# EricSteinberger/PokerRL

Measured on AMD Instinct MI355X. Metric: CFR+ node-updates/sec on FHP public tree, higher is better.
Workload: dtype f32

## Files before the change

include/pokerrl_hip.h:

```cpp
#ifndef POKERRL_HIP_H
#define POKERRL_HIP_H

#include <stdint.h>

#ifdef __cplusplus
extern "C" {
#endif

#define PRL_MAX_BET_SIZES 96

#define PRL_OK 0
#define PRL_ERR_ARG (-1)
#define PRL_ERR_NO_DEVICE (-2)
#define PRL_ERR_HIP (-3)
#define PRL_ERR_UNSUPPORTED (-4)
#define PRL_ERR_OOM (-5)
#define PRL_ERR_STATE (-6)

typedef struct PrlRules {
    int32_t n_hole_cards;
    int32_t n_ranks;
    int32_t n_suits;
    int32_t n_cards;
    int32_t range_size;
// ... 214 lines not shown
int32_t prl_solver_time_iterations_ex(prl_solver_t* solver, int32_t n, float* out_ms, float* out_pass_ms, int32_t* out_n_pass);

int32_t prl_solver_time_evaluations(prl_solver_t* solver, int32_t n, float* out_ms, float* out_pass_ms, int32_t* out_n_pass);

enum {
    PRL_SF_REACH = 0,
    PRL_SF_EV = 1,
    PRL_SF_EV_BR = 2,
    PRL_SF_STRATEGY = 3,
    PRL_SF_STRAT_F64 = 4,
    PRL_SF_REGRET = 5,
    PRL_SF_AVG = 6,
    PRL_SF_AVG_F64 = 7,
    PRL_SF_AVG_SUM = 8,
    PRL_SF_BR_IDX = 9,
    PRL_SF_EXPL_HISTORY = 10,
    PRL_SF_ITER = 11,
    PRL_SF_CONSTANTS = 12,
    PRL_SF_BYTES_ALLOCATED = 13,
    PRL_SF_ENGINE = 14,
    PRL_SF_GRAPH_REPLAY = 15,
    PRL_SF_EXCHANGES = 17,
    PRL_SF_VMM_RANGES = 18,
    PRL_SF_EXPLICIT_STRATEGY = 16
};
int32_t prl_solver_get(prl_solver_t* solver, int32_t field, void* out);
int32_t prl_solver_set_strategy_device(prl_solver_t* solver, const prl_tree_t* tree, const float* d_probs, int32_t n_actions);
int32_t prl_solver_get_cols(prl_solver_t* solver, int32_t field, int64_t col_begin, int64_t n_cols, void* out);

int32_t prl_lbr_checkdown_equity(const PrlRules* rules, const int8_t* board_dealt, int32_t n_dealt, const int8_t* lbr_hand,
                                 const float* ranges, int32_t n_q, float* out_wp);

int32_t prl_lbr_batch_run(const PrlGame* lbr_game, const PrlGame* agent_game, const PrlRules* rules, int32_t n_envs, int32_t agent_seat,
                          int32_t check_to_round, int32_t agent_kind, uint32_t agent_seed, uint32_t episode_base, double reward_scalar,
                          double ev_normalizer, const int8_t* cards, float* out_winnings, uint64_t* out_stats4, float* out_device_ms);

int32_t prl_h2h_batch_run(const PrlGame* game, const PrlRules* rules, int32_t n_envs, int32_t ref_seat, int32_t ref_kind, uint32_t ref_seed,
                          int32_t opp_kind, uint32_t opp_seed, uint32_t episode_base, double reward_scalar, double ev_normalizer,
                          const int8_t* cards, float* out_winnings, uint64_t* out_stats2, float* out_device_ms);

typedef struct PrlPolicyTable prl_policy_table_t;
prl_policy_table_t* prl_policy_table_create(const uint64_t* keys, const int32_t* rows, uint32_t capacity, const float* probs, int32_t n_rows,
                                            int32_t n_actions, int32_t range_size, uint32_t key_seed);
void prl_policy_table_destroy(prl_policy_table_t* table);
int32_t prl_policy_table_probe(const prl_policy_table_t* table, int32_t n, const uint32_t* key_lo, const uint32_t* key_hi, const int32_t* action,
                               const int32_t* hand, int32_t* out_row, float* out_prob);
// ... 23 lines not shown
```

pokerrl_amd/_native.py:

```python
import ctypes
import os

import numpy as np

_HERE = os.path.dirname(os.path.abspath(__file__))
EXCHANGE_FN = ctypes.CFUNCTYPE(ctypes.c_int32, ctypes.c_void_p, ctypes.c_void_p, ctypes.c_void_p, ctypes.c_uint64)
LIB_PATH = os.environ.get("POKERRL_AMD_LIB", os.path.join(_HERE, "lib", "libpokerrl_hip.so"))

PRL_MAX_BET_SIZES = 96


class NativeError(RuntimeError):
    status = None


ERR_ARG, ERR_NO_DEVICE, ERR_HIP, ERR_UNSUPPORTED, ERR_OOM, ERR_STATE = -1, -2, -3, -4, -5, -6


class PrlRules(ctypes.Structure):
    _fields_ = [
        ("n_hole_cards", ctypes.c_int32), ("n_ranks", ctypes.c_int32), ("n_suits", ctypes.c_int32),
        ("n_cards", ctypes.c_int32), ("range_size", ctypes.c_int32), ("n_rounds", ctypes.c_int32),
        ("board_cards_in_round", ctypes.c_int32 * 4), ("n_board_cards", ctypes.c_int32),
        ("btn_first_postflop", ctypes.c_int32), ("rank_rule", ctypes.c_int32),
# ... 499 lines not shown
        L.prl_tree_observations_device.restype = ctypes.c_int32
        check(L.prl_tree_observations_device(self._h, int(kind), 1 if invert else 0, _ptr(idx), _ptr(off), len(idx), None if fo is None else _ptr(fo),
                                              int(row_dim), int(n_rows), ctypes.c_void_p(int(d_out)), ctypes.c_void_p(int(d_legal or 0)), int(n_actions)), L)

    def obs_stats(self):
        out = np.zeros(4, np.float64)
        self._L.prl_tree_obs_stats.argtypes = [ctypes.c_void_p, ctypes.c_void_p]
        self._L.prl_tree_obs_stats.restype = ctypes.c_int32
        check(self._L.prl_tree_obs_stats(self._h, _ptr(out)), self._L)
        return dict(state_bytes=int(out[0]), states_ms=float(out[1]), obs_ms=float(out[2]), obs_bytes=int(out[3]))

    def __del__(self):
        try:
            if self._h:
                self._L.prl_tree_destroy(self._h)
                self._h = None
        except Exception:
            pass


OBS_VANILLA, OBS_HISTORY, OBS_FLAT_HU_LIMIT = 0, 1, 2

SF = dict(reach=0, ev=1, ev_br=2, strategy=3, strat_f64=4, regret=5, avg=6, avg_f64=7, avg_sum=8, br_idx=9,
          expl_history=10, iter=11, constants=12, bytes_allocated=13, engine=14, graph_replay=15, explicit_strategy=16, exchanges=17, vmm_ranges=18)
VARIANTS = {"vanilla": 0, "plus": 1, "linear": 2}
ENGINES = {"auto": 0, "levels": 1, "fused": 2}


class NativeSolver:

    def __init__(self, tree, variant, delay=0, engine="auto", _lib=None, shard=None, avg_dtype="f64", place=None, probe_iters=4, board_mult=None,
                 symmetrize=False):
        self._L = _lib or tree._L
        self.placement_ms, self.placement_chosen = None, None
        if _lib is None and self._L is lib():
            require_device()
        self.tree = tree
        self._h = ctypes.c_void_p()
        v = VARIANTS[variant] if isinstance(variant, str) else int(variant)
        e = ENGINES[engine] if isinstance(engine, str) else int(engine)
        self._exchange_cb = None
        if board_mult is not None and shard is not None:
            raise ValueError("weighted boards (board_mult=): one GPU -- not with shard=")
        if symmetrize and board_mult is None:
            raise ValueError("symmetrize= goes with board_mult= (suit-class representatives and their orbit sizes)")
        if shard is not None and isinstance(shard[0], str):
            assert shard[0] == "rccl"
# ... 210 lines not shown

        th = [threading.Thread(target=work, args=(n,), daemon=True) for n in names]
        for t in th:
            t.start()
        try:
            for c0 in range(0, self.n_cols, cols_per_piece):
                for n in names:
                    qs[n].put(self.get_cols(n, c0, min(cols_per_piece, self.n_cols - c0)))
        finally:
            for n in names:
                qs[n].put(None)
            for t in th:
                t.join()
        return {n: h.hexdigest() for n, h in hs.items()}

    def get(self, name):
        n, c, R = self.n_nodes, self.n_cols, self.R
        shape, dtype = {
            "reach": ((n, 2, R), np.float32), "ev": ((n, 2, R), np.float32), "ev_br": ((n, 2, R), np.float32),
            "strategy": ((c, R), np.float64), "strat_f64": ((n,), np.uint8), "regret": ((c, R), np.float32),
            "avg": ((c, R), np.float64), "avg_f64": ((n,), np.uint8), "avg_sum": ((c, R), np.float32),
            "br_idx": ((n, R), np.int32), "constants": ((2,), np.float32), "bytes_allocated": ((1,), np.int64),
            "explicit_strategy": ((1,), np.int32), "exchanges": ((1,), np.int64), "vmm_ranges": ((2,), np.int64),
        }.get(name, (None, None))
        if name == "expl_history":
            shape, dtype = (self.iter + 1, 2), np.float32
        out = np.zeros(shape, dtype)
        self._call("prl_solver_get", SF[name], _ptr(out))
        return out
```

pokerrl_amd/csrc/prl_fhp.h:

```cpp
#pragma once
#include "prl_defs.h"
#include "prl_solver_types.h"
#include "prl_tree.h"

enum { PRL_SRC_REGRET = 0, PRL_SRC_UNIFORM64 = 1, PRL_SRC_ARR64 = 2, PRL_SRC_ARR32 = 3,
       PRL_SRC_STRAT32 = 4 ,
       PRL_SRC_AVGF32 = 5  };
enum { PRL_FHP_UPDATE0 = 0, PRL_FHP_UPDATE1 = 1, PRL_FHP_EVAL = 2, PRL_FHP_UPDATE0_EVAL = 3, PRL_FHP_UPDATE0_BR = 4, PRL_FHP_UPDATE1_EVAL1 = 5,
       PRL_FHP_EVAL0 = 6 };
constexpr bool prl_fhp_runs_seat(int mode, int p) {
    return mode == PRL_FHP_EVAL || mode == PRL_FHP_UPDATE0_EVAL ? true
         : (mode == PRL_FHP_UPDATE1 || mode == PRL_FHP_UPDATE1_EVAL1) ? p == 1 : p == 0;
}
constexpr bool prl_fhp_updates(int mode, int p) {
    return p == 0 ? (mode == PRL_FHP_UPDATE0 || mode == PRL_FHP_UPDATE0_EVAL || mode == PRL_FHP_UPDATE0_BR)
                  : (mode == PRL_FHP_UPDATE1 || mode == PRL_FHP_UPDATE1_EVAL1);
}
constexpr bool prl_fhp_with_br(int mode) { return mode >= PRL_FHP_EVAL; }
constexpr int prl_fhp_out_width(int mode) {
    return mode == PRL_FHP_UPDATE1_EVAL1 ? 3
         : (prl_fhp_runs_seat(mode, 0) && prl_fhp_runs_seat(mode, 1) ? 2 : 1) * (prl_fhp_with_br(mode) ? 2 : 1);
}

#define PRL_FHP_MAX_NODES 40
// ... 85 lines not shown

struct PrlFhpShapeDesc {
    int32_t n_nodes, n_cols, n_dec;
    int32_t kind[PRL_FHP_MAX_NODES], actor[PRL_FHP_MAX_NODES], nch[PRL_FHP_MAX_NODES], parent[PRL_FHP_MAX_NODES], col0[PRL_FHP_MAX_NODES],
        folder[PRL_FHP_MAX_NODES];
    int32_t dec_nch[PRL_FHP_MAX_DEC], dec_col0[PRL_FHP_MAX_DEC];
};
template <class D>
inline PrlFhpShapeDesc prl_fhp_describe() {
    PrlFhpShapeDesc d = {};
    d.n_nodes = D::N_NODES; d.n_cols = D::N_COLS; d.n_dec = D::N_DEC;
    static_assert(D::N_NODES <= PRL_FHP_MAX_NODES && D::N_DEC <= PRL_FHP_MAX_DEC, "enlarge PRL_FHP_MAX_*");
    for (int n = 0; n < D::N_NODES; ++n) {
        d.kind[n] = D::kind(n); d.actor[n] = D::actor(n); d.nch[n] = D::nch(n); d.parent[n] = D::parent(n); d.col0[n] = D::col0(n);
        d.folder[n] = D::folder(n);
    }
    for (int j = 0; j < D::N_DEC; ++j) { d.dec_nch[j] = D::nch(D::dec_node(j)); d.dec_col0[j] = D::col0(D::dec_node(j)); }
    return d;
}
enum { PRL_FHP_SHAPE_15 = 0, PRL_FHP_SHAPE_9 = 1, PRL_FHP_SHAPE_21 = 2, PRL_FHP_N_SHAPES = 3 };
const PrlFhpShapeDesc& prl_fhp_shape_desc(int shape_id);

#define PRL_FHP_NP 1088
struct PrlFhpParams {
    int32_t n_boards, R;
    int32_t np;
    int32_t variant, iter;
    int32_t max_grid;
    int32_t shape;
    int32_t n_cols_board, n_dec;
    int32_t dec_nch[PRL_FHP_MAX_DEC], dec_col0[PRL_FHP_MAX_DEC];
    float chance_prob, eq_const;
    float pot[PRL_FHP_MAX_NODES];
    const float* chance_reach;
    const float* board_w;
    float* regret;
    double* avg;
    float* avg32;
    int32_t avg_mode;
    double m_old, m_new;
    float* avg_sum;
    int32_t avgsum_mask, avgsum_iter[2];
    int32_t block_sum;
    int32_t exp;
    int32_t no_steady;
    const double* strat_arr;
    float* board_out;
    const int16_t* plan_pp;
    const uint32_t* plan_clx;
    unsigned long long* timing;
};

int prl_fhp_match_shape(const PrlFlatTree& t, int* chance_node, int* first_board_node, int* col_base, float* pots );

int prl_launch_fhp_pass(const PrlFhpParams& prm, int mode, int src0, int src1, void* stream);
void prl_launch_fhp_strategy_from_regret(const PrlFhpParams& prm, double* out_region, void* stream);
void prl_launch_fhp_avg_from_sum(const PrlFhpParams& prm, void* stream);
void prl_launch_fhp_symmetrize(const float* in, int n_vec, int R, const int32_t* class_of, const int32_t* class_start, const int32_t* class_hands, float* out, void* stream);
void prl_launch_fhp_expand(const PrlFhpParams& prm, const void* region, int elem, int b0, int nb, const void* fill_by_col, const void* blocked_src,
                           void* dst, void* stream);
void prl_launch_fhp_compact(const PrlFhpParams& prm, const void* src, int elem, int b0, int nb, void* region, void* blocked_dst, void* stream);
#define PRL_FHP_NBLOCKED (1326 - 1081)
void prl_launch_fhp_chance_sum(const float* d_board_vals, int n_boards, int W, float* d_scratch, float* d_dest, void* stream);
// ... 6 lines not shown
```

pokerrl_amd/csrc/prl_fhp_pass.inc:

```
#ifndef FHP_NPAD
#define FHP_NPAD 1088
#define FHP_NLIVE 1081
#define FHP_NCARDS 52
#define FHP_R 1326
#define FHP_NP PRL_FHP_NP
#define FHP_NSHOW (PrlFhpShape::N_SHOW)
#define FHP_NFOLD (PrlFhpShape::N_FOLD)
#define FHP_NVEC (PrlFhpShape::N_SHOW + PrlFhpShape::N_FOLD)
#endif
typedef PrlFhpDerive<FHP_SPEC> PrlFhpShape;
#if defined(FHP_EXPERIMENT)
#define FHP_EXP(c, bit) (((c).prm->exp & (bit)) != 0)
#define FHP_AVG_PIPELINED(c) true
#define FHP_TERMINAL_CACHE(c) true
#else
#define FHP_EXP(c, bit) false
#define FHP_AVG_PIPELINED(c) true
#define FHP_TERMINAL_CACHE(c) true
#endif
static_assert(PrlFhpShape::subtree_size(0) == PrlFhpShape::N_NODES, "the spec is one DFS pre-order tree");
static_assert(FHP_NP == FHP_NPAD && FHP_NP == PRL_PP_NPAD && FHP_R == PRL_PP_R && FHP_SLOTS == 2, "sorted storage: a column holds the padded sorted domain, a lane two positions");

#include "prl_fhp_div.inc"
struct FhpV { FhpF v; };
// ... 138 lines not shown
    return -1;
}
constexpr int FHP_PF_RG_ROWS = fhp_seat_rows(0) > fhp_seat_rows(1) ? fhp_seat_rows(0) : fhp_seat_rows(1);
#define FHP_PF_RG_WORDS (FHP_PF_RG_ROWS * 256)
#define FHP_LDS_WORK_BYTES ((FHP_NVEC * FHP_NPAD + 2 * FHP_NSHOW * FHP_NPAD + FHP_NFOLD * 64 + 16 + FHP_ACC_WORDS) * 4)
#define FHP_LDS_BYTES_WITH_RG (FHP_LDS_WORK_BYTES + (FHP_PF_RG_WORDS + FHP_PF_AREA(PRL_CLX_WORDS) + FHP_PF_AREA(FHP_PP_WORDS)) * 4)
#define FHP_RG_IN_LDS (FHP_LDS_BYTES_WITH_RG <= 160 * 1024)
#define FHP_LDS_BYTES (FHP_RG_IN_LDS ? FHP_LDS_BYTES_WITH_RG : FHP_LDS_BYTES_WITH_RG - FHP_PF_RG_WORDS * 4)

PRL_DEV PRL_INLINE FhpLds fhp_lds() {
    FhpLds L;
    float* f = (float*)prl_smem();
    L.y = f; f += FHP_NVEC * FHP_NPAD;
    L.K = f; f += 2 * FHP_NSHOW * FHP_NPAD;
    L.Tc = f; f += FHP_NFOLD * 64;
    L.Tt = f; f += 16;
    L.acc = f; f += FHP_ACC_WORDS;
    L.pf_rg = f; f += FHP_RG_IN_LDS ? FHP_PF_RG_WORDS : 0;
    L.pf_clx = (uint32_t*)f; f += FHP_PF_AREA(PRL_CLX_WORDS);
    L.pf_pp = (uint32_t*)f; f += FHP_PF_AREA(FHP_PP_WORDS);
    return L;
}

template <int STEADY>
struct FhpCtxT {
    static constexpr bool own_after_b(int src_opp) { return src_opp == PRL_SRC_REGRET && !(STEADY == 1 || STEADY == 4); }
    PRL_DEV PRL_INLINE int variant() const {
        if constexpr (STEADY == 1 || STEADY == 4) return PRL_CFR_PLUS;
        else if constexpr (STEADY == 2) return PRL_CFR_LINEAR;
        else if constexpr (STEADY == 3) return PRL_CFR_VANILLA;
        else return variant_;
    }
    PRL_DEV PRL_INLINE bool first_iteration() const { if constexpr (STEADY != 0) return false; else return iter == 0; }
    PRL_DEV PRL_INLINE int avg_mode() const { if constexpr (STEADY == 1 || STEADY == 4) return 2; else if constexpr (STEADY >= 2) return 0; else return prm->avg_mode; }
    PRL_DEV PRL_INLINE int avgsum_mask() const { if constexpr (STEADY == 1 || STEADY == 4) return 0; else return prm->avgsum_mask; }
    PRL_DEV PRL_INLINE bool avg32() const { if constexpr (STEADY == 4) return true; else if constexpr (STEADY != 0) return false; else return prm->avg32 != nullptr; }
    FhpLds L;
    int wave;
    uint32_t pf_lds;
    uint32_t rec0, rec1;
    int p0;
    int gsm1[FHP_SLOTS];
    int gem1[FHP_SLOTS];
    bool live[FHP_SLOTS];
    int c1[FHP_SLOTS], c2[FHP_SLOTS];
    int sh[FHP_SLOTS];
    bool active;
    bool valid;
    float eq_const;
    int variant_, iter;
    const PrlFhpParams* prm;
    size_t cofs;
    FhpF nr0, nr1;
    float nw;
    double av_old[PrlFhpShape::N_COLS][FHP_SLOTS];
    bool fast;
#ifdef PRL_FHP_TIMING
    long long t_prev, t_acc[6];
// ... 355 lines not shown
                        fhp_gstore_nt(c.prm->regret + c.cofs + (size_t)(col0 + i) * FHP_NP, rn[i]);
                    }
                    constexpr bool KEEP = MODE == PRL_FHP_UPDATE1_EVAL1;
                    if (KEEP || c.avg_mode()) {
                        float t[3][FHP_SLOTS], sum[FHP_SLOTS];
                        for (int k = 0; k < FHP_SLOTS; ++k) {
                            sum[k] = 0.f;
                            for (int i = 0; i < A; ++i) {
                                t[i][k] = c.variant() == PRL_CFR_PLUS ? rn[i][k] : (rn[i][k] > 0.f ? rn[i][k] : 0.f);
                                sum[k] = sum[k] + t[i][k];
                            }
                        }
                        float qn[3][FHP_SLOTS];
#if !defined(FHP_DIV_FAST) || defined(FHP_NEWSTRAT_GENERIC)
                        fhp_regret_match<A>(t, sum, qn, false);
#else
                        fhp_regret_match<A>(t, sum, qn, prl_ballot(!fhp_node_in_box<A>(t, sum)) == 0ull);
#endif
                        for (int i = 0; i < A; ++i) {
                            double an[FHP_SLOTS];
                            for (int k = 0; k < FHP_SLOTS; ++k) {
                                const float sn = qn[i][k];
                                if (KEEP) R.rg[col0 + i][k] = sn;
                                an[k] = c.avg_mode() == 2 ? c.prm->m_old * c.av_old[col0 + i][k] + c.prm->m_new * (double)sn : (double)sn;
                            }
                            if (c.avg_mode()) {
                                if (c.avg32()) {
                                    float af[FHP_SLOTS];
                                    for (int k = 0; k < FHP_SLOTS; ++k) af[k] = (float)an[k];
                                    fhp_gstore_nt(c.prm->avg32 + c.cofs + (size_t)(col0 + i) * FHP_NP, af);
                                } else fhp_gstore_nt(c.prm->avg + c.cofs + (size_t)(col0 + i) * FHP_NP, an);
                            }
                        }
                    }
                    if (c.avg_mode() == 2 && FHP_AVG_PIPELINED(c)) fhp_request_old_average<fhp_node_of_rank(P, fhp_completion_rank(P, NODE) + 2)>(c);
                }
            } else {
                FhpF acc = ce[0].v, accb = cb[0].v;
                for (int i = 1; i < A; ++i) { acc = acc + ce[i].v; accb = accb + cb[i].v; }
                ev.v = acc;
                br.v = accb;
            }
        }
    }
};

struct FhpSrc { const float* rg; const uint32_t* clx; const int16_t* pp; };
// ... 294 lines not shown
    }
    if (prm.block_sum && b_begin < b_end) {
        prl_sync_lds();
        flush_block((b_end - 1) / PRL_CHANCE_BLOCK);
    }
#ifdef PRL_FHP_TIMING
    if (tid == 0) for (int i = 0; i < 6; ++i) atomicAdd(prm.timing + i, (unsigned long long)c.t_acc[i]);
#endif
}

template <int MODE, int S0, int S1, int STEADY = 0>
static void fhp_launch_t(const PrlFhpParams& prm, int grid, void* stream) {
    PRL_LAUNCH((prl_k_fhp_pass<MODE, S0, S1, STEADY>), grid, FHP_THREADS, FHP_LDS_BYTES, stream, prm);
}

int launch_pass(const PrlFhpParams& prm, int mode, int src0, int src1, void* stream) {
    if (prm.n_boards <= 0) return PRL_OK;
    if (prm.R != FHP_R) return PRL_ERR_UNSUPPORTED;
    if (((prm.avgsum_mask & 1) && src0 != PRL_SRC_REGRET) || ((prm.avgsum_mask & 2) && src1 != PRL_SRC_REGRET)) return PRL_ERR_UNSUPPORTED;
    static_assert(FHP_NVEC <= 16 && FHP_LDS_BYTES <= 160 * 1024, "terminal vectors + prefetch area of this shape must fit the CU's LDS");
    int grid = prm.n_boards < prm.max_grid ? prm.n_boards : prm.max_grid;
    const int key = mode * 100 + src0 * 10 + src1;
    const int steady = prm.no_steady || prm.iter == 0 ? 0
                       : (prm.variant == PRL_CFR_PLUS && prm.avg_mode == 2 && prm.avgsum_mask == 0) ? (prm.avg32 ? 4 : 1)
                       : (prm.variant == PRL_CFR_LINEAR && prm.avg_mode == 0) ? 2
                       : (prm.variant == PRL_CFR_VANILLA && prm.avg_mode == 0) ? 3 : 0;
    switch (key) {
        case PRL_FHP_UPDATE0 * 100 + PRL_SRC_UNIFORM64 * 10 + PRL_SRC_UNIFORM64: fhp_launch_t<PRL_FHP_UPDATE0, PRL_SRC_UNIFORM64, PRL_SRC_UNIFORM64>(prm, grid, stream); break;
        case PRL_FHP_UPDATE1 * 100 + PRL_SRC_REGRET * 10 + PRL_SRC_UNIFORM64: fhp_launch_t<PRL_FHP_UPDATE1, PRL_SRC_REGRET, PRL_SRC_UNIFORM64>(prm, grid, stream); break;
        case PRL_FHP_UPDATE0 * 100 + PRL_SRC_REGRET * 10 + PRL_SRC_REGRET: fhp_launch_t<PRL_FHP_UPDATE0, PRL_SRC_REGRET, PRL_SRC_REGRET>(prm, grid, stream); break;
        case PRL_FHP_UPDATE1 * 100 + PRL_SRC_REGRET * 10 + PRL_SRC_REGRET: fhp_launch_t<PRL_FHP_UPDATE1, PRL_SRC_REGRET, PRL_SRC_REGRET>(prm, grid, stream); break;
        case PRL_FHP_UPDATE0_EVAL * 100 + PRL_SRC_REGRET * 10 + PRL_SRC_REGRET: fhp_launch_t<PRL_FHP_UPDATE0_EVAL, PRL_SRC_REGRET, PRL_SRC_REGRET>(prm, grid, stream); break;
        case PRL_FHP_UPDATE0_BR * 100 + PRL_SRC_REGRET * 10 + PRL_SRC_REGRET:
            if (steady == 1) fhp_launch_t<PRL_FHP_UPDATE0_BR, PRL_SRC_REGRET, PRL_SRC_REGRET, 1>(prm, grid, stream);
            else if (steady == 4) fhp_launch_t<PRL_FHP_UPDATE0_BR, PRL_SRC_REGRET, PRL_SRC_REGRET, 4>(prm, grid, stream);
            else if (steady == 2) fhp_launch_t<PRL_FHP_UPDATE0_BR, PRL_SRC_REGRET, PRL_SRC_REGRET, 2>(prm, grid, stream);
            else if (steady == 3) fhp_launch_t<PRL_FHP_UPDATE0_BR, PRL_SRC_REGRET, PRL_SRC_REGRET, 3>(prm, grid, stream);
            else fhp_launch_t<PRL_FHP_UPDATE0_BR, PRL_SRC_REGRET, PRL_SRC_REGRET>(prm, grid, stream);
            break;
        case PRL_FHP_UPDATE1_EVAL1 * 100 + PRL_SRC_REGRET * 10 + PRL_SRC_REGRET:
            if (steady == 1) fhp_launch_t<PRL_FHP_UPDATE1_EVAL1, PRL_SRC_REGRET, PRL_SRC_REGRET, 1>(prm, grid, stream);
            else if (steady == 4) fhp_launch_t<PRL_FHP_UPDATE1_EVAL1, PRL_SRC_REGRET, PRL_SRC_REGRET, 4>(prm, grid, stream);
            else if (steady == 2) fhp_launch_t<PRL_FHP_UPDATE1_EVAL1, PRL_SRC_REGRET, PRL_SRC_REGRET, 2>(prm, grid, stream);
            else if (steady == 3) fhp_launch_t<PRL_FHP_UPDATE1_EVAL1, PRL_SRC_REGRET, PRL_SRC_REGRET, 3>(prm, grid, stream);
            else fhp_launch_t<PRL_FHP_UPDATE1_EVAL1, PRL_SRC_REGRET, PRL_SRC_REGRET>(prm, grid, stream);
            break;
        case PRL_FHP_EVAL0 * 100 + PRL_SRC_REGRET * 10 + PRL_SRC_REGRET: fhp_launch_t<PRL_FHP_EVAL0, PRL_SRC_REGRET, PRL_SRC_REGRET>(prm, grid, stream); break;
        case PRL_FHP_EVAL * 100 + PRL_SRC_UNIFORM64 * 10 + PRL_SRC_UNIFORM64: fhp_launch_t<PRL_FHP_EVAL, PRL_SRC_UNIFORM64, PRL_SRC_UNIFORM64>(prm, grid, stream); break;
        case PRL_FHP_EVAL * 100 + PRL_SRC_REGRET * 10 + PRL_SRC_REGRET: fhp_launch_t<PRL_FHP_EVAL, PRL_SRC_REGRET, PRL_SRC_REGRET>(prm, grid, stream); break;
        case PRL_FHP_EVAL * 100 + PRL_SRC_ARR64 * 10 + PRL_SRC_ARR64: fhp_launch_t<PRL_FHP_EVAL, PRL_SRC_ARR64, PRL_SRC_ARR64>(prm, grid, stream); break;
        case PRL_FHP_EVAL * 100 + PRL_SRC_STRAT32 * 10 + PRL_SRC_STRAT32: fhp_launch_t<PRL_FHP_EVAL, PRL_SRC_STRAT32, PRL_SRC_STRAT32>(prm, grid, stream); break;
        case PRL_FHP_EVAL * 100 + PRL_SRC_AVGF32 * 10 + PRL_SRC_AVGF32: fhp_launch_t<PRL_FHP_EVAL, PRL_SRC_AVGF32, PRL_SRC_AVGF32>(prm, grid, stream); break;
        case PRL_FHP_EVAL * 100 + PRL_SRC_ARR32 * 10 + PRL_SRC_ARR32: fhp_launch_t<PRL_FHP_EVAL, PRL_SRC_ARR32, PRL_SRC_ARR32>(prm, grid, stream); break;
        default: return PRL_ERR_UNSUPPORTED;
    }
    return PRL_OK;
}
```

pokerrl_amd/csrc/prl_solver.hip:

```cpp
#include <math.h>
#include <stdlib.h>
#include <string.h>
#if !defined(PRL_EMU)
#include <dlfcn.h>
#include <rccl/rccl.h>
#endif

#include <algorithm>
#include <string>
#include <unordered_map>
#include <vector>

#include "prl_cards.h"
#include "prl_device.h"
#include "prl_fhp.h"
#include "prl_host.h"
#include "prl_kernels.h"
#include "prl_policy.h"
#include "prl_rt.h"
#include "prl_solver_types.h"
#include "prl_st.h"

#define PRL_NODE_LEAF 4

// ... 34 lines not shown
    const float* d_board_w = nullptr;
    bool symmetrize = false;
    float* d_row_sym = nullptr;
    const int32_t *d_sym_class_of = nullptr, *d_sym_class_start = nullptr, *d_sym_class_hands = nullptr;
    float* d_half = nullptr;
    PrlIterDev* d_ip = nullptr;
    const int32_t* d_level_start = nullptr;
    bool small_tree = false;
    void* levels_graph_exec = nullptr;
    bool graphs_off = false;
    int avg_pending[2] = {-1, -1};
    bool time_passes = false;
    std::vector<hipEvent_t> pass_events;
    bool expl_pending = false;
    PrlFhpParams fp{};
    int chance_trunk = -1;
    float* d_sum_scratch = nullptr;
    double* d_user_strategy = nullptr;
    float* d_user_strategy32 = nullptr;
    int user_strategy_f64 = -1;
    int src[2] = {PRL_SRC_UNIFORM64, PRL_SRC_UNIFORM64};
    bool board_avg_f64 = false;
    bool board_avg_stale = false;
    float* d_regret = nullptr;
    double* d_avg = nullptr;
    float* d_avg32 = nullptr;
    bool avg_f32 = false;
    long long n_exchanges = 0;
    void* rccl_comm = nullptr;
    bool streets = false;
    PrlStPlanHost st;
    PrlStParams sp{};
    struct StLevelDev { PrlStInst* inst = nullptr; } st_dev[PRL_ST_MAX_GROUPS];
    struct StStreetDev { float* leaf_reach = nullptr; float* val = nullptr; } st_str[PRL_ST_MAX_LEVELS + 1];
    PrlFlatTree chain_ft;
    PrlDevTree Tc{};
    float* d_chain_ev = nullptr;
    PrlStChainTerm* d_chain_terms = nullptr;
    PrlStChainBundle* d_chain_bundles = nullptr;
    hipStream_t chain_stream = nullptr;
    hipEvent_t chain_fork = nullptr, chain_join = nullptr;
    std::vector<int32_t> chain_level_start;
    int n_chain_term = 0, n_chain_bundles = 0, n_chain = 0;
    PrlStChainDev chain_dev{};
    int32_t* d_trunk_leaves = nullptr;
    int n_trunk_leaves = 1;
    std::vector<int32_t> col_dfs;
    std::vector<int32_t> col_int;
    bool sorted = false;
    int col_base = 0, ncb = 0;
    size_t board_ofs = 0, col_elems = 0;
// ... 256 lines not shown
    PRL_HIP_TRY(hipMemsetAsync(st->reach, 0, nv * sizeof(float), s->stream));
    PRL_HIP_TRY(hipMemsetAsync(st->ev, 0, nv * sizeof(float), s->stream));
    PRL_HIP_TRY(hipMemsetAsync(st->ev_br, 0, nv * sizeof(float), s->stream));
    return PRL_OK;
}

float chance_prob_f32(int n_children, int n_cards, int n_hole, int n_dealt) {
    double denom = (double)n_children * (double)prl_comb(n_cards - 2 * n_hole, n_dealt) / (double)prl_comb(n_cards, n_dealt);
    return (float)(1.0 / denom);
}
float eq_const_f32(int n_cards, int n_hole) {
    return (float)((double)prl_comb(n_cards, n_hole) / (double)prl_comb(n_cards - n_hole, n_hole));
}

int do_update_reach(prl_solver* s, const PrlDevState& st) {
    bool& root_set = &st == &s->S ? s->root_reach_set[0] : s->root_reach_set[1];
    prl_launch_reach(s->T, st, s->ft.level_start.data(), s->stream, root_set && &st == &s->S);
    root_set = true;
    PRL_HIP_TRY(hipGetLastError());
    return PRL_OK;
}

static int ensure_board_avg(prl_solver* s) {
    if (!s->fused || !s->board_avg_stale) return PRL_OK;
    if (s->streets) {
        for (int lv = 0; lv < s->st.n_groups; ++lv) {
            PrlStParams q = s->sp;
            q.n_inst = s->st.group[lv].n_inst; q.col_base = s->st.group[lv].col_base; q.avg_sum = s->S.avg_sum; q.avg = s->d_avg;
            prl_launch_st_avg_from_sum(q, s->st.group[lv].spec, s->stream);
        }
        PRL_HIP_TRY(hipGetLastError());
        s->board_avg_stale = false;
        return PRL_OK;
    }
    PrlFhpParams p = s->fp;
    p.avg_sum = s->S.avg_sum + s->board_ofs;
    p.avg = s->d_avg + s->board_ofs;
    prl_launch_fhp_avg_from_sum(p, s->stream);
    PRL_HIP_TRY(hipGetLastError());
    s->board_avg_stale = false;
    return PRL_OK;
}

int street_sweep(prl_solver* s, const PrlDevState& st, int mode, int src0, int src1, const double* strat_arr, const float* strat32) {
    PrlStParams p = s->sp;
    p.regret = strat32 ? const_cast<float*>(strat32) : s->d_regret;
// ... 1161 lines not shown
        return PRL_ERR_STATE;
    }
    if (h.fingerprint != s->fingerprint) {
        prl_set_error("load_state: the blob belongs to another board list / game / stack sizes or to another rank's shard");
        return PRL_ERR_STATE;
    }
    if (h.src0 < 0 || h.src0 > PRL_SRC_ARR32 || h.src1 < 0 || h.src1 > PRL_SRC_ARR32) { prl_set_error("load_state: corrupt header"); return PRL_ERR_ARG; }
    const StateLayout L = state_layout(s, h.iter);
    if (bytes < L.total) { prl_set_error("load_state: truncated blob"); return PRL_ERR_ARG; }
    const char* b = (const char*)in;
    const size_t nc = col_array_elems(s), tc = (size_t)s->T.n_cols * s->R;
    TRY(ensure_hist(s, h.iter + 1));
    PRL_HIP_TRY(hipStreamSynchronize(s->stream));
    PRL_HIP_TRY(hipMemcpy(s->d_regret, b + L.regret, nc * 4, hipMemcpyHostToDevice));
    PRL_HIP_TRY(hipMemcpy(s->d_avg, b + L.avg, nc * 8, hipMemcpyHostToDevice));
    if (s->S.avg_sum) PRL_HIP_TRY(hipMemcpy(s->S.avg_sum, b + L.avg_sum, nc * 4, hipMemcpyHostToDevice));
    PRL_HIP_TRY(hipMemcpy(s->S.strategy, b + L.strategy, tc * 8, hipMemcpyHostToDevice));
    PRL_HIP_TRY(hipMemcpy(s->S.strat_f64, b + L.strat_f64, (size_t)s->T.n_nodes, hipMemcpyHostToDevice));
    PRL_HIP_TRY(hipMemcpy(s->S.avg_f64, b + L.avg_f64, (size_t)s->T.n_nodes, hipMemcpyHostToDevice));
    PRL_HIP_TRY(hipMemcpy(s->d_expl_hist, b + L.hist, (size_t)(h.iter + 1) * 2 * 4, hipMemcpyHostToDevice));
    s->iter = h.iter; s->src[0] = h.src0; s->src[1] = h.src1; s->board_avg_f64 = h.board_avg_f64 != 0; s->board_avg_stale = false;
    s->user_strategy_f64 = -1; s->expl_pending = false; s->have_half = false; s->avg_pending[0] = s->avg_pending[1] = -1;
    s->ev_valid = false;
    for (double& a : s->blk_avg) a = 0.;
    for (int it = 0; it < s->iter; ++it) {
        int mode; double m_old, m_new;
        cfr_plus_weights(s, it, &mode, &m_old, &m_new);
        blocked_avg_step(s, mode, m_old, m_new);
    }
    return do_update_reach(s, s->S);
}

int32_t prl_solver_get_stream(prl_solver_t* s, void** out) {
    if (!s || !out) { prl_set_error("NULL argument"); return PRL_ERR_ARG; }
    *out = (void*)s->stream;
    return PRL_OK;
}

int32_t prl_solver_set_exchange_async(prl_solver_t* s, int32_t on) {
    if (!s) { prl_set_error("NULL solver"); return PRL_ERR_ARG; }
    s->exchange_async = on != 0;
    return PRL_OK;
}

int32_t prl_chance_sum_host_ragged(const float* board_values, int32_t n_boards, int32_t R, int32_t world, int32_t shard_boards, float* out) {
    if (!board_values || !out || n_boards <= 0 || R <= 0 || world < 1 || shard_boards <= 0 || (int64_t)(world - 1) * shard_boards >= n_boards ||
// ... 53 lines not shown
    for (void* r : s->vmm) { vmm_free(*(PrlVmmRange*)r); delete (PrlVmmRange*)r; }
#endif
    if (s->chain_fork) (void)hipEventDestroy(s->chain_fork);
    if (s->chain_join) (void)hipEventDestroy(s->chain_join);
    if (s->chain_stream) (void)hipStreamDestroy(s->chain_stream);
    if (s->stream) (void)hipStreamDestroy(s->stream);
    delete s;
}

int32_t prl_solver_reset(prl_solver_t* s) {
    if (!s) { prl_set_error("NULL solver"); return PRL_ERR_ARG; }
    const size_t nc = col_array_elems(s);
    s->iter = 0;
    for (double& a : s->blk_avg) a = 0.;
    s->expl_pending = false;
    s->have_half = false;
    s->avg_pending[0] = s->avg_pending[1] = -1;
    PRL_HIP_TRY(hipMemsetAsync(s->d_regret, 0, nc * sizeof(float), s->stream));
    PRL_HIP_TRY(hipMemsetAsync(s->d_avg, 0, (s->avg_f32 ? (size_t)s->T.n_cols * s->R : nc) * sizeof(double), s->stream));
    if (s->avg_f32) PRL_HIP_TRY(hipMemsetAsync(s->d_avg32, 0, nc * sizeof(float), s->stream));
    PRL_HIP_TRY(hipMemsetAsync(s->S.avg_f64, 0, (size_t)s->T.n_nodes, s->stream));
    if (s->S.avg_sum) PRL_HIP_TRY(hipMemsetAsync(s->S.avg_sum, 0, nc * sizeof(float), s->stream));
    s->board_avg_f64 = false; s->board_avg_stale = false;
    TRY(prl_solver_fill_uniform(s));
    TRY(ensure_ev(s));
    return record_expl(s);
}

int32_t prl_solver_fill_uniform(prl_solver_t* s) {
    if (!s) { prl_set_error("NULL solver"); return PRL_ERR_ARG; }
    PRL_HIP_TRY(hipMemsetAsync(s->S.strat_f64, 0, (size_t)s->T.n_nodes, s->stream));
    prl_launch_fill_uniform(s->T, s->S, s->d_col_node, s->stream);
    s->src[0] = s->src[1] = PRL_SRC_UNIFORM64;
    s->user_strategy_f64 = -1;
    s->have_half = false;
    s->ev_valid = false;
    return do_update_reach(s, s->S);
}

int32_t prl_solver_set_strategy(prl_solver_t* s, const void* strat, int32_t is_f64) {
    return prl_solver_set_strategy_mixed(s, strat, is_f64, nullptr);
}

int32_t prl_solver_set_strategy_mixed(prl_solver_t* s, const void* strat, int32_t is_f64, const uint8_t* node_is_f64) {
    if (!s || !strat) { prl_set_error("NULL argument"); return PRL_ERR_ARG; }
    if (node_is_f64 && (!is_f64 || s->fused)) { prl_set_error("per-node strategy dtypes: float64 data, LEVELS engine"); return PRL_ERR_ARG; }
// ... 38 lines not shown
        }
        s->user_strategy_f64 = is_f64 ? 1 : 0;
    }
    PRL_HIP_TRY(hipMemcpyAsync(s->S.strategy, src, (size_t)s->T.n_cols * s->R * sizeof(double), hipMemcpyHostToDevice, s->stream));
    if (node_is_f64) PRL_HIP_TRY(hipMemcpyAsync(s->S.strat_f64, node_is_f64, (size_t)s->T.n_nodes, hipMemcpyHostToDevice, s->stream));
    else PRL_HIP_TRY(hipMemsetAsync(s->S.strat_f64, is_f64 ? 1 : 0, (size_t)s->T.n_nodes, s->stream));
    PRL_HIP_TRY(hipStreamSynchronize(s->stream));
    s->ev_valid = false;
    return do_update_reach(s, s->S);
}

int32_t prl_solver_update_reach(prl_solver_t* s) {
    if (!s) { prl_set_error("NULL solver"); return PRL_ERR_ARG; }
    s->ev_valid = false;
    return do_update_reach(s, s->S);
}

int32_t prl_solver_compute_ev(prl_solver_t* s) {
    if (!s) { prl_set_error("NULL solver"); return PRL_ERR_ARG; }
    s->ev_valid = false;
    return ensure_ev(s);
}

static int iteration_core(prl_solver* s, bool closing_eval) {
    if (s->fused && s->user_strategy_f64 >= 0) { prl_set_error("call reset() / fill_uniform() before iterating after set_strategy()"); return PRL_ERR_STATE; }
    int mode = 0;
    double m_old = 0., m_new = 0.;
    cfr_plus_weights(s, s->iter, &mode, &m_old, &m_new);
    s->fp.avg_mode = mode;
    s->fp.m_old = m_old;
    s->fp.m_new = m_new;
    for (int p = 0; p < 2; ++p) {
        bool second_half = false;
        if (s->fused) {
            const bool steady = s->src[0] == PRL_SRC_REGRET && s->src[1] == PRL_SRC_REGRET;
            if (p == 0 && s->expl_pending && s->have_half) {
                TRY(expl_to_history(s));
                TRY(do_compute_ev(s, s->S, PRL_FHP_UPDATE0_BR));
                s->expl_pending = false;
                s->have_half = false;
            } else if (p == 0 && s->expl_pending) {
                TRY(expl_to_history(s));
                TRY(do_compute_ev(s, s->S, PRL_FHP_UPDATE0_EVAL));
                s->expl_pending = false;
            } else if (p == 1 && steady) {
                TRY(do_compute_ev(s, s->S, PRL_FHP_UPDATE1_EVAL1));
                second_half = true;
            } else TRY(do_compute_ev(s, s->S, p == 0 ? PRL_FHP_UPDATE0 : PRL_FHP_UPDATE1));
        } else TRY(ensure_ev(s));
        prl_launch_regret_strategy(s->T, s->S, s->d_nodes_p[p], s->n_nodes_p[p], p, s->variant, s->iter, s->stream);
        s->src[p] = PRL_SRC_REGRET;
        s->ev_valid = false;
        TRY(do_update_reach(s, s->S));
        prl_launch_average(s->T, s->S, s->d_nodes_p[p], s->n_nodes_p[p], p, s->variant, s->iter, mode, m_old, m_new, s->stream);
        if (s->fused && mode) s->board_avg_f64 = mode == 2;
        if (s->fused && s->variant != PRL_CFR_PLUS) s->avg_pending[p] = s->iter;
        if (second_half) s->have_half = true;
    }
    s->fp.avg_mode = 0;
    if (s->sorted) blocked_avg_step(s, mode, m_old, m_new);
    s->iter += 1;
    if (s->fused && !closing_eval) {
        s->expl_pending = true;
        PRL_HIP_TRY(hipGetLastError());
        return PRL_OK;
    }
    if (s->fused && s->have_half) {
        TRY(do_compute_ev(s, s->S, PRL_FHP_EVAL0));
        s->have_half = false;
        s->ev_valid = true;
    } else TRY(ensure_ev(s));
    PRL_HIP_TRY(hipGetLastError());
    return record_expl(s);
}

static int small_tree_iterations(prl_solver* s, int n) {
    TRY(ensure_ev(s));
    TRY(ensure_hist(s, s->iter + n + 1));
    if (!s->d_ip) TRY(dev_alloc(s, &s->d_ip, (size_t)1));
    if (!s->d_level_start) TRY(dev_upload(s, &s->d_level_start, s->ft.level_start));
    PrlIterDev ip;
    memset(&ip, 0, sizeof(ip));
// ... 108 lines not shown
    for (int i = 0; i < n; ++i) PRL_HIP_TRY(hipGraphLaunch((hipGraphExec_t)s->levels_graph_exec, s->stream));
    s->iter += n;
    s->src[0] = s->src[1] = PRL_SRC_REGRET;
    s->ev_valid = true;
    PRL_HIP_TRY(hipGetLastError());
    return PRL_OK;
}
#endif

int32_t prl_solver_iteration(prl_solver_t* s) {
    if (!s) { prl_set_error("NULL solver"); return PRL_ERR_ARG; }
    return prl_solver_iterations(s, 1);
}

int32_t prl_solver_iterations(prl_solver_t* s, int32_t n) {
    if (!s) { prl_set_error("NULL solver"); return PRL_ERR_ARG; }
    if (!s->fused && s->small_tree && n > 0) return small_tree_iterations(s, n);
#if !defined(PRL_EMU)
    if (!s->fused && !s->graphs_off && n > 0) {
        const int rc = levels_graph_iterations(s, n);
        if (rc != PRL_ERR_UNSUPPORTED) return rc;
    }
#endif
    for (int i = 0; i < n; ++i) TRY(iteration_core(s, i == n - 1));
    return PRL_OK;
}

int32_t prl_solver_time_iterations_ex(prl_solver_t* s, int32_t n, float* out_ms, float* out_pass_ms, int32_t* out_n_pass) {
    if (!s || !out_ms || n < 0) { prl_set_error("bad argument"); return PRL_ERR_ARG; }
    hipEvent_t e0, e1;
    PRL_HIP_TRY(hipEventCreate(&e0));
    PRL_HIP_TRY(hipEventCreate(&e1));
    TRY(ensure_hist(s, s->iter + n + 1));
    s->time_passes = s->fused && out_pass_ms != nullptr;
    PRL_HIP_TRY(hipEventRecord(e0, s->stream));
    int rc = prl_solver_iterations(s, n);
    s->time_passes = false;
    if (rc == PRL_OK) {
        PRL_HIP_TRY(hipEventRecord(e1, s->stream));
        PRL_HIP_TRY(hipEventSynchronize(e1));
        PRL_HIP_TRY(hipEventElapsedTime(out_ms, e0, e1));
        float pass_ms = 0.f;
        const bool dump = getenv("PRL_DUMP_PASS_MS") != nullptr;
        for (size_t i = 0; i + 1 < s->pass_events.size(); i += 2) {
            float t = 0.f;
            PRL_HIP_TRY(hipEventElapsedTime(&t, s->pass_events[i], s->pass_events[i + 1]));
            pass_ms += t;
// ... 297 lines not shown
                    if (c < s->T.n_cols) memcpy(dst, tr.data() + (size_t)c * s->R, (size_t)s->R * 8);
                    else for (int h = 0; h < s->R; ++h) dst[h] = (double)f[(size_t)c * s->R + h];
                }
                return PRL_OK;
            }
            TRY(ensure_board_avg(s)); src = s->d_avg; bytes = nc * 8; break;
        case PRL_SF_AVG_F64: src = s->S.avg_f64; bytes = (size_t)s->T.n_nodes; break;
        case PRL_SF_AVG_SUM:
            if (s->sorted && s->S.avg_sum) {
                const size_t tcb = (size_t)s->T.n_cols * s->R;
                PRL_HIP_TRY(hipMemcpyAsync(out, s->S.avg_sum, tcb * 4, hipMemcpyDeviceToHost, s->stream));
                TRY(sorted_get_boards(s, s->S.avg_sum + s->board_ofs, 4, nullptr, nullptr, (float*)out + tcb, 4, 0, s->fp.n_boards));
                return prl_solver_sync(s);
            }
            src = s->S.avg_sum; bytes = nc * 4; break;
        case PRL_SF_BR_IDX: TRY(ensure_ev(s)); src = s->S.br_idx; bytes = (size_t)s->T.n_nodes * s->T.R * 4; break;
        case PRL_SF_EXPL_HISTORY: src = s->d_expl_hist; bytes = (size_t)(s->iter + 1) * 2 * 4; break;
        case PRL_SF_ITER: *(int32_t*)out = s->iter; return PRL_OK;
        case PRL_SF_CONSTANTS: ((float*)out)[0] = s->T.chance_prob; ((float*)out)[1] = s->T.eq_const; return PRL_OK;
        case PRL_SF_BYTES_ALLOCATED: *(int64_t*)out = (int64_t)s->bytes_allocated; return PRL_OK;
        case PRL_SF_ENGINE: *(int32_t*)out = s->fused ? PRL_ENGINE_FUSED : PRL_ENGINE_LEVELS; return PRL_OK;
        case PRL_SF_GRAPH_REPLAY: *(int32_t*)out = s->levels_graph_exec != nullptr; return PRL_OK;
        case PRL_SF_EXCHANGES: *(int64_t*)out = (int64_t)s->n_exchanges; return PRL_OK;
        case PRL_SF_VMM_RANGES: {
            int64_t bytes = 0;
#if !defined(PRL_EMU)
            for (void* r : s->vmm) bytes += (int64_t)((PrlVmmRange*)r)->size;
#endif
            ((int64_t*)out)[0] = (int64_t)s->vmm.size(); ((int64_t*)out)[1] = bytes; return PRL_OK;
        }
        case PRL_SF_EXPLICIT_STRATEGY: *(int32_t*)out = s->fused ? s->user_strategy_f64 : -1; return PRL_OK;
        default: prl_set_error("unknown solver field"); return PRL_ERR_ARG;
    }
    if (!src) { prl_set_error("field not available for this variant"); return PRL_ERR_STATE; }
    const bool col_field = field == PRL_SF_STRATEGY || field == PRL_SF_REGRET || field == PRL_SF_AVG || field == PRL_SF_AVG_SUM;
    if (col_field && !s->col_dfs.empty()) {
        std::vector<char> tmp(bytes);
        PRL_HIP_TRY(hipMemcpyAsync(tmp.data(), src, bytes, hipMemcpyDeviceToHost, s->stream));
        TRY(prl_solver_sync(s));
        const size_t cb = bytes / (size_t)s->full_cols;
        for (int c = 0; c < s->full_cols; ++c) memcpy((char*)out + (size_t)s->col_dfs[c] * cb, tmp.data() + (size_t)c * cb, cb);
        return PRL_OK;
    }
    PRL_HIP_TRY(hipMemcpyAsync(out, src, bytes, hipMemcpyDeviceToHost, s->stream));
    return prl_solver_sync(s);
}
// ... 279 lines not shown
```

Measured before the change: 178.6 million.

## Pair CFR+ average-strategy updates across two iterations to halve average traffic

In fused CFR+ mode, iterations are now processed in pairs. The first iteration skips the f64 average-strategy read-modify-write. The second applies both blends at once, folding the previous iteration's weighted strategy (recomputed from the pre-update regrets) into the old average before the current blend. This targets the per-iteration global-memory traffic on the f64 average buffer, paid for with two new kernel specialisations, extra register and arithmetic work in the catch-up pass, and a state flag that blocks reading the average while a pair is incomplete. The pairing can be disabled through an environment variable, and a counter for completed pairs is exposed.

```diff
diff --git a/include/pokerrl_hip.h b/include/pokerrl_hip.h
--- a/include/pokerrl_hip.h
+++ b/include/pokerrl_hip.h
@@ -260,6 +260,7 @@
     PRL_SF_GRAPH_REPLAY = 15,
     PRL_SF_EXCHANGES = 17,
     PRL_SF_VMM_RANGES = 18,
+    PRL_SF_AVG_PAIRS = 19,
     PRL_SF_EXPLICIT_STRATEGY = 16
 };
 int32_t prl_solver_get(prl_solver_t* solver, int32_t field, void* out);
diff --git a/pokerrl_amd/_native.py b/pokerrl_amd/_native.py
--- a/pokerrl_amd/_native.py
+++ b/pokerrl_amd/_native.py
@@ -545,7 +545,7 @@
 OBS_VANILLA, OBS_HISTORY, OBS_FLAT_HU_LIMIT = 0, 1, 2
 
 SF = dict(reach=0, ev=1, ev_br=2, strategy=3, strat_f64=4, regret=5, avg=6, avg_f64=7, avg_sum=8, br_idx=9,
-          expl_history=10, iter=11, constants=12, bytes_allocated=13, engine=14, graph_replay=15, explicit_strategy=16, exchanges=17, vmm_ranges=18)
+          expl_history=10, iter=11, constants=12, bytes_allocated=13, engine=14, graph_replay=15, explicit_strategy=16, exchanges=17, vmm_ranges=18, avg_pairs=19)
 VARIANTS = {"vanilla": 0, "plus": 1, "linear": 2}
 ENGINES = {"auto": 0, "levels": 1, "fused": 2}
 
@@ -802,6 +802,7 @@
             "avg": ((c, R), np.float64), "avg_f64": ((n,), np.uint8), "avg_sum": ((c, R), np.float32),
             "br_idx": ((n, R), np.int32), "constants": ((2,), np.float32), "bytes_allocated": ((1,), np.int64),
             "explicit_strategy": ((1,), np.int32), "exchanges": ((1,), np.int64), "vmm_ranges": ((2,), np.int64),
+            "avg_pairs": ((1,), np.int64),
         }.get(name, (None, None))
         if name == "expl_history":
             shape, dtype = (self.iter + 1, 2), np.float32
diff --git a/pokerrl_amd/csrc/prl_fhp.h b/pokerrl_amd/csrc/prl_fhp.h
--- a/pokerrl_amd/csrc/prl_fhp.h
+++ b/pokerrl_amd/csrc/prl_fhp.h
@@ -131,6 +131,7 @@
 const PrlFhpShapeDesc& prl_fhp_shape_desc(int shape_id);
 
 #define PRL_FHP_NP 1088
+enum { PRL_FHP_AVG_NORMAL = 0, PRL_FHP_AVG_DEFERRED = 1, PRL_FHP_AVG_CATCH_UP = 2 };
 struct PrlFhpParams {
     int32_t n_boards, R;
     int32_t np;
@@ -148,6 +149,8 @@
     float* avg32;
     int32_t avg_mode;
     double m_old, m_new;
+    int32_t avg_pair;
+    double m_old_prev, m_new_prev;
     float* avg_sum;
     int32_t avgsum_mask, avgsum_iter[2];
     int32_t block_sum;
diff --git a/pokerrl_amd/csrc/prl_fhp_pass.inc b/pokerrl_amd/csrc/prl_fhp_pass.inc
--- a/pokerrl_amd/csrc/prl_fhp_pass.inc
+++ b/pokerrl_amd/csrc/prl_fhp_pass.inc
@@ -184,18 +184,24 @@
     return L;
 }
 
+constexpr bool fhp_steady_plus(int steady) { return steady == 1 || steady == 4 || steady == 5 || steady == 6; }
 template <int STEADY>
 struct FhpCtxT {
-    static constexpr bool own_after_b(int src_opp) { return src_opp == PRL_SRC_REGRET && !(STEADY == 1 || STEADY == 4); }
+    static constexpr bool own_after_b(int src_opp) { return src_opp == PRL_SRC_REGRET && !fhp_steady_plus(STEADY); }
     PRL_DEV PRL_INLINE int variant() const {
-        if constexpr (STEADY == 1 || STEADY == 4) return PRL_CFR_PLUS;
+        if constexpr (fhp_steady_plus(STEADY)) return PRL_CFR_PLUS;
         else if constexpr (STEADY == 2) return PRL_CFR_LINEAR;
         else if constexpr (STEADY == 3) return PRL_CFR_VANILLA;
         else return variant_;
     }
     PRL_DEV PRL_INLINE bool first_iteration() const { if constexpr (STEADY != 0) return false; else return iter == 0; }
-    PRL_DEV PRL_INLINE int avg_mode() const { if constexpr (STEADY == 1 || STEADY == 4) return 2; else if constexpr (STEADY >= 2) return 0; else return prm->avg_mode; }
-    PRL_DEV PRL_INLINE int avgsum_mask() const { if constexpr (STEADY == 1 || STEADY == 4) return 0; else return prm->avgsum_mask; }
+    PRL_DEV PRL_INLINE int avg_mode() const {
+        if constexpr (STEADY == 1 || STEADY == 4 || STEADY == 6) return 2;
+        else if constexpr (STEADY != 0) return 0;
+        else return prm->avg_pair == PRL_FHP_AVG_DEFERRED ? 0 : prm->avg_mode;
+    }
+    PRL_DEV PRL_INLINE bool avg_catch_up() const { if constexpr (STEADY == 6) return true; else if constexpr (STEADY != 0) return false; else return prm->avg_pair == PRL_FHP_AVG_CATCH_UP; }
+    PRL_DEV PRL_INLINE int avgsum_mask() const { if constexpr (fhp_steady_plus(STEADY)) return 0; else return prm->avgsum_mask; }
     PRL_DEV PRL_INLINE bool avg32() const { if constexpr (STEADY == 4) return true; else if constexpr (STEADY != 0) return false; else return prm->avg32 != nullptr; }
     FhpLds L;
     int wave;
@@ -597,7 +603,11 @@
                             for (int k = 0; k < FHP_SLOTS; ++k) {
                                 const float sn = qn[i][k];
                                 if (KEEP) R.rg[col0 + i][k] = sn;
-                                an[k] = c.avg_mode() == 2 ? c.prm->m_old * c.av_old[col0 + i][k] + c.prm->m_new * (double)sn : (double)sn;
+                                double ao = c.av_old[col0 + i][k];
+                                if constexpr (SRC == PRL_SRC_REGRET) {
+                                    if (c.avg_catch_up()) ao = c.prm->m_old_prev * ao + c.prm->m_new_prev * (double)s[i][k];
+                                }
+                                an[k] = c.avg_mode() == 2 ? c.prm->m_old * ao + c.prm->m_new * (double)sn : (double)sn;
                             }
                             if (c.avg_mode()) {
                                 if (c.avg32()) {
@@ -938,7 +948,8 @@
     int grid = prm.n_boards < prm.max_grid ? prm.n_boards : prm.max_grid;
     const int key = mode * 100 + src0 * 10 + src1;
     const int steady = prm.no_steady || prm.iter == 0 ? 0
-                       : (prm.variant == PRL_CFR_PLUS && prm.avg_mode == 2 && prm.avgsum_mask == 0) ? (prm.avg32 ? 4 : 1)
+                       : (prm.variant == PRL_CFR_PLUS && prm.avg_mode == 2 && prm.avgsum_mask == 0)
+                           ? (prm.avg32 ? 4 : prm.avg_pair == PRL_FHP_AVG_DEFERRED ? 5 : prm.avg_pair == PRL_FHP_AVG_CATCH_UP ? 6 : 1)
                        : (prm.variant == PRL_CFR_LINEAR && prm.avg_mode == 0) ? 2
                        : (prm.variant == PRL_CFR_VANILLA && prm.avg_mode == 0) ? 3 : 0;
     switch (key) {
@@ -950,6 +961,8 @@
         case PRL_FHP_UPDATE0_BR * 100 + PRL_SRC_REGRET * 10 + PRL_SRC_REGRET:
             if (steady == 1) fhp_launch_t<PRL_FHP_UPDATE0_BR, PRL_SRC_REGRET, PRL_SRC_REGRET, 1>(prm, grid, stream);
             else if (steady == 4) fhp_launch_t<PRL_FHP_UPDATE0_BR, PRL_SRC_REGRET, PRL_SRC_REGRET, 4>(prm, grid, stream);
+            else if (steady == 5) fhp_launch_t<PRL_FHP_UPDATE0_BR, PRL_SRC_REGRET, PRL_SRC_REGRET, 5>(prm, grid, stream);
+            else if (steady == 6) fhp_launch_t<PRL_FHP_UPDATE0_BR, PRL_SRC_REGRET, PRL_SRC_REGRET, 6>(prm, grid, stream);
             else if (steady == 2) fhp_launch_t<PRL_FHP_UPDATE0_BR, PRL_SRC_REGRET, PRL_SRC_REGRET, 2>(prm, grid, stream);
             else if (steady == 3) fhp_launch_t<PRL_FHP_UPDATE0_BR, PRL_SRC_REGRET, PRL_SRC_REGRET, 3>(prm, grid, stream);
             else fhp_launch_t<PRL_FHP_UPDATE0_BR, PRL_SRC_REGRET, PRL_SRC_REGRET>(prm, grid, stream);
@@ -957,6 +970,8 @@
         case PRL_FHP_UPDATE1_EVAL1 * 100 + PRL_SRC_REGRET * 10 + PRL_SRC_REGRET:
             if (steady == 1) fhp_launch_t<PRL_FHP_UPDATE1_EVAL1, PRL_SRC_REGRET, PRL_SRC_REGRET, 1>(prm, grid, stream);
             else if (steady == 4) fhp_launch_t<PRL_FHP_UPDATE1_EVAL1, PRL_SRC_REGRET, PRL_SRC_REGRET, 4>(prm, grid, stream);
+            else if (steady == 5) fhp_launch_t<PRL_FHP_UPDATE1_EVAL1, PRL_SRC_REGRET, PRL_SRC_REGRET, 5>(prm, grid, stream);
+            else if (steady == 6) fhp_launch_t<PRL_FHP_UPDATE1_EVAL1, PRL_SRC_REGRET, PRL_SRC_REGRET, 6>(prm, grid, stream);
             else if (steady == 2) fhp_launch_t<PRL_FHP_UPDATE1_EVAL1, PRL_SRC_REGRET, PRL_SRC_REGRET, 2>(prm, grid, stream);
             else if (steady == 3) fhp_launch_t<PRL_FHP_UPDATE1_EVAL1, PRL_SRC_REGRET, PRL_SRC_REGRET, 3>(prm, grid, stream);
             else fhp_launch_t<PRL_FHP_UPDATE1_EVAL1, PRL_SRC_REGRET, PRL_SRC_REGRET>(prm, grid, stream);
diff --git a/pokerrl_amd/csrc/prl_solver.hip b/pokerrl_amd/csrc/prl_solver.hip
--- a/pokerrl_amd/csrc/prl_solver.hip
+++ b/pokerrl_amd/csrc/prl_solver.hip
@@ -80,11 +80,13 @@
     int src[2] = {PRL_SRC_UNIFORM64, PRL_SRC_UNIFORM64};
     bool board_avg_f64 = false;
     bool board_avg_stale = false;
+    bool avg_deferred = false;
     float* d_regret = nullptr;
     double* d_avg = nullptr;
     float* d_avg32 = nullptr;
     bool avg_f32 = false;
     long long n_exchanges = 0;
+    long long n_avg_pairs = 0;
     void* rccl_comm = nullptr;
     bool streets = false;
     PrlStPlanHost st;
@@ -387,6 +389,7 @@
 }
 
 static int ensure_board_avg(prl_solver* s) {
+    if (s->avg_deferred) { prl_set_error("the board average is incomplete: an iteration failed between the two halves of a paired average update; reset() or load_state()"); return PRL_ERR_STATE; }
     if (!s->fused || !s->board_avg_stale) return PRL_OK;
     if (s->streets) {
         for (int lv = 0; lv < s->st.n_groups; ++lv) {
@@ -1594,6 +1597,7 @@
     s->iter = h.iter; s->src[0] = h.src0; s->src[1] = h.src1; s->board_avg_f64 = h.board_avg_f64 != 0; s->board_avg_stale = false;
     s->user_strategy_f64 = -1; s->expl_pending = false; s->have_half = false; s->avg_pending[0] = s->avg_pending[1] = -1;
     s->ev_valid = false;
+    s->avg_deferred = false;
     for (double& a : s->blk_avg) a = 0.;
     for (int it = 0; it < s->iter; ++it) {
         int mode; double m_old, m_new;
@@ -1693,6 +1697,7 @@
     PRL_HIP_TRY(hipMemsetAsync(s->S.avg_f64, 0, (size_t)s->T.n_nodes, s->stream));
     if (s->S.avg_sum) PRL_HIP_TRY(hipMemsetAsync(s->S.avg_sum, 0, nc * sizeof(float), s->stream));
     s->board_avg_f64 = false; s->board_avg_stale = false;
+    s->avg_deferred = false;
     TRY(prl_solver_fill_uniform(s));
     TRY(ensure_ev(s));
     return record_expl(s);
@@ -1777,7 +1782,7 @@
     return ensure_ev(s);
 }
 
-static int iteration_core(prl_solver* s, bool closing_eval) {
+static int iteration_core(prl_solver* s, bool closing_eval, int avg_pair = PRL_FHP_AVG_NORMAL) {
     if (s->fused && s->user_strategy_f64 >= 0) { prl_set_error("call reset() / fill_uniform() before iterating after set_strategy()"); return PRL_ERR_STATE; }
     int mode = 0;
     double m_old = 0., m_new = 0.;
@@ -1785,6 +1790,14 @@
     s->fp.avg_mode = mode;
     s->fp.m_old = m_old;
     s->fp.m_new = m_new;
+    s->fp.avg_pair = avg_pair;
+    s->fp.m_old_prev = s->fp.m_new_prev = 0.;
+    if (avg_pair == PRL_FHP_AVG_CATCH_UP) {
+        int mode_prev = 0;
+        cfr_plus_weights(s, s->iter - 1, &mode_prev, &s->fp.m_old_prev, &s->fp.m_new_prev);
+        if (mode_prev != 2 || mode != 2) { prl_set_error("paired average update outside the blending iterations"); return PRL_ERR_STATE; }
+    }
+    if (avg_pair == PRL_FHP_AVG_DEFERRED) s->avg_deferred = true;
     for (int p = 0; p < 2; ++p) {
         bool second_half = false;
         if (s->fused) {
@@ -1813,6 +1826,8 @@
         if (second_half) s->have_half = true;
     }
     s->fp.avg_mode = 0;
+    s->fp.avg_pair = PRL_FHP_AVG_NORMAL;
+    if (avg_pair == PRL_FHP_AVG_CATCH_UP) { s->avg_deferred = false; ++s->n_avg_pairs; }
     if (s->sorted) blocked_avg_step(s, mode, m_old, m_new);
     s->iter += 1;
     if (s->fused && !closing_eval) {
@@ -1967,7 +1982,20 @@
         if (rc != PRL_ERR_UNSUPPORTED) return rc;
     }
 #endif
-    for (int i = 0; i < n; ++i) TRY(iteration_core(s, i == n - 1));
+    if (s->avg_deferred) { prl_set_error("an iteration failed between the two halves of a paired average update; reset() or load_state()"); return PRL_ERR_STATE; }
+    const bool may_pair = s->fused && !s->streets && s->variant == PRL_CFR_PLUS && !s->avg_f32 && !getenv("PRL_FHP_NO_AVG_PAIR");
+    bool deferred = false;
+    for (int i = 0; i < n; ++i) {
+        int avg_pair = PRL_FHP_AVG_NORMAL;
+        if (deferred) avg_pair = PRL_FHP_AVG_CATCH_UP;
+        else if (may_pair && i + 1 < n && s->src[0] == PRL_SRC_REGRET && s->src[1] == PRL_SRC_REGRET && s->user_strategy_f64 < 0) {
+            int mode; double m_old, m_new;
+            cfr_plus_weights(s, s->iter, &mode, &m_old, &m_new);
+            if (mode == 2) avg_pair = PRL_FHP_AVG_DEFERRED;
+        }
+        TRY(iteration_core(s, i == n - 1, avg_pair));
+        deferred = avg_pair == PRL_FHP_AVG_DEFERRED;
+    }
     return PRL_OK;
 }
 
@@ -2311,6 +2339,7 @@
         case PRL_SF_ENGINE: *(int32_t*)out = s->fused ? PRL_ENGINE_FUSED : PRL_ENGINE_LEVELS; return PRL_OK;
         case PRL_SF_GRAPH_REPLAY: *(int32_t*)out = s->levels_graph_exec != nullptr; return PRL_OK;
         case PRL_SF_EXCHANGES: *(int64_t*)out = (int64_t)s->n_exchanges; return PRL_OK;
+        case PRL_SF_AVG_PAIRS: *(int64_t*)out = (int64_t)s->n_avg_pairs; return PRL_OK;
         case PRL_SF_VMM_RANGES: {
             int64_t bytes = 0;
 #if !defined(PRL_EMU)
```

New measurement: 194.5 million, median of 6. 8.9% higher.
